# FlowEternal/multitask-hydranet

Measured on AMD Instinct MI355X. Metric: images/sec (fwd+bwd) HydraNet @ default res, 1/2/4/8 MI355X; CPU-ref same run, higher is better.
Workload: dtype bf16; 1 GPU; full HydraNet (backbone + BiFPN + seg/det/lane heads + multitask loss), big cfg, fwd+loss+bwd; batch_per_gpu=16, global_batch=16, resolution=3x512x1024, parallelism=dp1, hipgraph=True

## Files before the change

include/hydranet_hip.h:

```cpp
#ifndef HYDRANET_HIP_H
#define HYDRANET_HIP_H

#ifdef __cplusplus
extern "C" {
#endif

typedef struct ihipStream_t* hipStream_t;


int hn_gconv_pack_diag(const float* w, void* wk, void* wd, int C, hipStream_t stream);
int hn_pack_weight(const float* w, void* wp, void* wt, int Cout, int Cin, int taps, hipStream_t stream);
int hn_pack_weight_ex(const float* w, void* wp, void* wt, int Cout, int Cin_total, int ci0, int Cin, int taps, int phase, const float* bias,
                      float* b_eff, hipStream_t stream);
int hn_phase_fold(const float* dw_eff, const float* dw1, const float* db_eff, float* dw, float* db, int K, int C0, int C1, hipStream_t stream);
int hn_pack_weights_batched(const long* jobs, int njobs, long total_blocks, const int* block_job, hipStream_t stream);
int hn_pack_small_batched(const long* jobs, const int* block_job, long total_blocks, hipStream_t stream);

int hn_conv_gemm_nt(const void* x0, const void* x1, int mode, int n_img, int H, int W, int C0, int C1, int ld0, int ld1, int up, long M,
                    const void* w, int Nout, int KP, int taps, const float* bias, int act, void* out, int out_f32, int ldc, long rpi,
                    long img_stride, float* psum, float* psq, hipStream_t stream);
int hn_nt_stat_rows(long M, int Nout);
int hn_nt_stat_tile(long M, int Nout);
int hn_direct_stat_rows(int n_img, int H, int W);
int hn_conv_gemm_nt_imgw(const void* x0, int ld0, long M, int C0, const void* w, long w_img_stride, long rows_per_image, int Nout, int KP,
                         const float* bias, int act, void* out, int ldc, const void* addend, int ld_add, hipStream_t stream);
int hn_scale_weight_gate(const void* wp, const float* gate, void* out, int N, int Cout, int C, int KP, hipStream_t stream);
int hn_conv_gemm_nt_lvl(const void* x0, int ld0, long M, int C0, const void* w, int Nout, int KP, const float* bias, int act, void* out,
                        int ldc, const float* coef, int nlev, const long* rows, hipStream_t stream);
int hn_conv_gemm_nt_lvlout(const void* x0, int ld0, long M, int C0, const void* w, int Nout, int KP, const float* bias, int act, float* out,
                           int ldc, long img_stride, int n_img, int nlev, const int* H, const int* W, int row_align, hipStream_t stream);

int hn_conv_gemm_nt_ex(const void* x0, const void* x1, int mode, int n_img, int H, int W, int C0, int C1, int ld0, int ld1, int up, long M,
                       const void* w, int Nout, int KP, int taps, const float* bias, int act, void* out, int out_f32, int ldc, long rpi,
                       long img_stride, float* psum, float* psq, const float* xscale, const float* xshift, const float* xgate, long xhw,
                       int xact, const void* addend, int ld_add, int add_mode, hipStream_t stream);
int hn_conv_gemm_nt_stat(const void* x0, const void* x1, int mode, int n_img, int H, int W, int C0, int C1, int ld0, int ld1, int up, long M,
                         const void* w, int Nout, int KP, int taps, const float* bias, int act, void* out, int out_f32, int ldc, long rpi,
                         long img_stride, float* psum, float* psq, const void* addend, int ld_add, int add_mode, int emode, const void* ez,
                         int ld_ez, const float* ecoef, hipStream_t stream);
int hn_conv_gemm_nt_stat3(const void* x0, int ld0, long M, int C0, const void* w, int Nout, int KP, void* out, int ldc, float* psum, float* psq,
                          const void* addend, int ld_add, const void* ez, int ld_ez, const void* ey, int ld_ey, const float* ecoef,
                          hipStream_t stream);
int hn_wgrad_plan(int mode, int n_img, int H, int W, long M, int Nout, int KP, int taps, int* splits, long* rows_per_split, long* ws_bytes);
int hn_conv_gemm_tn(const void* x0, const void* x1, int mode, int n_img, int H, int W, int C0, int C1, int ld0, int ld1, int up, long M,
                    const void* dz, int ldz, int Nout, int KP, int taps, float* workspace, float* dw, hipStream_t stream);


int hn_stem_fwd(const float* x, const float* w, void* z, void* patches, int N, int H, int W, hipStream_t stream);

int hn_gconv_pack(const float* w, void* wk, void* wd, int C, int flip, hipStream_t stream);
int hn_gconv_fwd(const void* in, int ldi, const void* wk, void* out, int ldo, int N, int Hi, int Wi, int C, int stride, hipStream_t stream);
int hn_gconv_dgrad_s2(const void* dz, int ldz, const void* wd, void* dx, int ldx, int N, int Hi, int Wi, int C, hipStream_t stream);
long hn_wgrad_chunks(long pixels, long items);
int hn_gconv_wgrad(const void* x, int ldx, const void* dz, int ldz, float* part, int N, int Hi, int Wi, int C, int stride,
                   hipStream_t stream);

int hn_dw_pack(const float* w, void* wk, void* wkf, int C, hipStream_t stream);
int hn_dwconv_fwd(const void* in, int ldi, const void* wk, void* out, int ldo, int N, int H, int W, int C, hipStream_t stream);
int hn_dwconv_fwd_levels(const void* in, int ldi, const void* wk, void* out, int ldo, int N, int C, int nlev, const int* H, const int* W,
                         int row_align, int accumulate, hipStream_t stream);
long hn_dwconv_wgrad_blocks(long strips, int C);
int hn_dwconv_wgrad(const void* x, int ldx, const void* dz, int ldz, float* part, int N, int H, int W, int C, hipStream_t stream);
int hn_dwconv_wgrad_levels(const void* x, int ldx, const void* dz, int ldz, float* part, int N, int C, int nlev, const int* H, const int* W,
                           int row_align, hipStream_t stream);
long hn_dwconv_bwd_blocks(long strips, int C);
long hn_dwconv_bwd_blocks_levels(int N, int C, int nlev, const int* H, const int* W);
int hn_dwconv_bwd_levels(const void* dz, int ldz, const void* x, int ldx, const void* wf, void* dx, int lddx, float* part, int N, int C,
                         int nlev, const int* H, const int* W, int row_align, int accumulate, hipStream_t stream);

int hn_maxpool_fwd(const void* in, int ldi, void* out, int ldo, int N, int H, int W, int C, int mode, hipStream_t stream);
int hn_maxpool_bwd(const void* in, int ldi, const void* dout, int ldd, void* dx, int ldx, const float* wscale, int N, int H, int W, int C,
                   int mode, hipStream_t stream);
int hn_maxpool_bwd2(const void* in, int ldi, const void* dout, int ldd, void* dx, int ldx, const float* wscale, void* arg_ws, int N, int H,
                    int W, int C, int mode, int accumulate, hipStream_t stream);

int hn_up2_fwd(const void* in, int ldi, void* out, int ldo, int N, int H, int W, int C, hipStream_t stream);
int hn_sum2x2(const void* g, int ldg, void* out, int ldo, const float* wscale, int N, int H, int W, int C, int accumulate, hipStream_t stream);

int hn_fuse_dweights(const float* pw, int blocks, const float* praw, int nw, float eps, float* dp, hipStream_t stream);
int hn_fuse_fwd(const void* const* in, const int* ld, const int* mode, const float* w, void* out, int ldo, int N, int H, int W, int C,
                hipStream_t stream);
int hn_fuse_fwd_raw(const void* const* in, const int* ld, const int* mode, const float* praw, int nw, float eps, float* wn, void* out, int ldo,
                    int N, int H, int W, int C, hipStream_t stream);
int hn_fuse_bwd_blocks(int N, int H, int W, int C);
int hn_fuse_bwd(const void* const* in, const int* ld, const int* mode, const float* w, const void* dout, int ldd, void* g, int ldg,
                void* const* din, const int* ldin, const int* acc, float* pw, int N, int H, int W, int C, hipStream_t stream);
int hn_fuse_bwd_arg(const void* const* in, const int* ld, const int* mode, const float* w, const void* dout, int ldd, void* g, int ldg,
                    void* const* din, const int* ldin, const int* acc, float* pw, void* const* arg_out, int N, int H, int W, int C,
                    hipStream_t stream);
int hn_maxpool_bwd_from_arg(const void* arg, const void* dout, int ldd, void* dx, int ldx, const float* wscale, int N, int H, int W, int C,
                            int mode, int accumulate, hipStream_t stream);

long hn_fold_ring_rows(int H, int W);
int hn_conv3x3_dgrad_fold(const void* dz, int ldz, int Cz, int n_img, int H, int W, const void* wt, int Nout, int KP, int phase_k, int clamp,
                          void* out, int ldo, const void* yprev, int ldy, void* ring, hipStream_t stream);
int hn_conv3x3_dgrad_fold_s2d(const void* dz, int ldz, int Cz, int n_img, int H, int W, const void* wt, int Nout, int KP, int phase_k, int clamp,
                              void* out, int ldo, void* out_s2d, int ld_s2d, const void* yprev, int ldy, void* ring, hipStream_t stream);
int hn_seg_fold(const void* dvp, int ldv, int c0, void* out, int ldo, const void* yprev, int ldy, int N, int H, int W, int C, int up,
                hipStream_t stream);

int hn_space_to_depth(const float* dy, void* out, int ldo, int N, int h, int w, int k, hipStream_t stream);

int hn_space_to_depth_blocks(int N, int h, int w, int k);
int hn_space_to_depth_bf16(const void* in, int ldi, void* out, int N, int h, int w, int k, float* psum, hipStream_t stream);

int hn_conv3x3_phase(const void* x0, int mode, int n_img, int H, int W, int C0, int ld0, const void* w, int Nout, int KP, const float* bias,
                     int act, void* out, int ldc, int k, const void* addend, int ld_add, hipStream_t stream);
int hn_conv3x3_out_argmax(const void* x0, int n_img, int H, int W, int C0, int ld0, const void* w, int k, int KP, const float* bias, long* mask,
                          hipStream_t stream);
int hn_wgrad_plan_phase(int n_img, int H, int W, int Nout, int KP, int phase_span, int* splits, long* rows_per_split, long* ws_bytes);
int hn_conv_gemm_tn_phase(const void* x0, int n_img, int H, int W, int C0, int ld0, const void* dz, int ldz, int Nout, int KP, int phase_span,
                          float* workspace, float* dw, float* dbias_eff, hipStream_t stream);
int hn_conv_gemm_tn_deferred(const void* x0, const void* x1, int mode, int n_img, int H, int W, int C0, int C1, int ld0, int ld1, int up, long M,
                             const void* dz, int ldz, int Nout, int KP, int taps, float* workspace, float* dw, long* job, hipStream_t stream);
int hn_wgrad_reduce_jobs(const long* jobs, int njobs, hipStream_t stream);
long hn_gconv_wgrad_group_ws_bytes(const long* jobs, int njobs);
int hn_gconv_wgrad_group(const long* jobs, int njobs, float* workspace, hipStream_t stream);

int hn_grad_tail(const long* jobs, int njobs, hipStream_t stream);

long hn_wgrad_group_ws_bytes(const long* jobs, int njobs);
int hn_wgrad_group(const long* jobs, int njobs, float* workspace, hipStream_t stream);

int hn_conv_gemm_tn_bias(const void* x0, const void* x1, int mode, int n_img, int H, int W, int C0, int C1, int ld0, int ld1, int up, long M,
                         const void* dz, int ldz, int Nout, int KP, int taps, float* workspace, float* dw, float* dbias, hipStream_t stream);

int hn_head_grad(const float* dy, const float* y, long rpi, long img_stride, int lds, int Nout, void* dz, int ldz, long M, int sigmoid,
                 hipStream_t stream);

int hn_pack_levels(const void* const* src, const int* ld, void* dst, int ldd, int N, int C, int nlev, const int* H, const int* W, int row_align,
                   hipStream_t stream);
int hn_head_grad_levels(const float* dy, const float* y, long img_stride, int lds, int Nout, void* dz, int ldz, int N, int nlev, const int* H,
                        const int* W, int row_align, int sigmoid, hipStream_t stream);


long hn_colred_rows(long M, long align);
int hn_col_stats(const void* x, int ldx, long M, int C, long R, float* psum, float* psq, hipStream_t stream);
int hn_col_dot(const void* a, int lda, const void* b, int ldb, long M, int C, long R, float* pdot, float* psum, hipStream_t stream);
int hn_rows_reduce(const float* in, float* out, int G, int S, int C, float alpha, hipStream_t stream);
int hn_rows_reduce2(const float* in1, const float* in2, float* out1, float* out2, int rows, int G, int C, hipStream_t stream);

int hn_bn_finalize(const float* psum, const float* psq, int prows, int C, long count, const float* gamma, const float* beta, float eps,
                   float momentum, float* running_mean, float* running_var, float* scale, float* shift, float* mean, float* rstd,
                   hipStream_t stream);
int hn_bn_eval_coeff(const float* gamma, const float* beta, const float* rm, const float* rv, float eps, int C, float* scale, float* shift,
                     hipStream_t stream);
int hn_bn_act(const void* z, int ldz, const float* scale, const float* shift, const void* res, int ldr, const float* rscale,
              const float* rshift, int act, void* out, int ldo, long M, int C, hipStream_t stream);
int hn_bn_bwd_reduce(const void* dout, int ldd, const void* z, int ldz, const void* y, int ldy, const float* scale, const float* shift,
                     const float* mean, const float* rstd, int act, long M, int C, long R, float* pg, float* pgx, hipStream_t stream);
int hn_bn_bwd_finalize(const float* pg, const float* pgx, int prows, int C, long count, float* dgamma, float* dbeta, float* mg, float* mgx,
                       hipStream_t stream);
int hn_bn_bwd_apply(const void* dout, int ldd, const void* z, int ldz, const void* y, int ldy, const float* scale, const float* shift,
                    const float* mean, const float* rstd, const float* mg, const float* mgx, int act, void* dz, int lddz, void* gout, int ldg,
                    long M, int C, hipStream_t stream);

dgamma/dbeta are HOST arrays of nlev device pointers.  Partial-row inputs hold one row per `div` tensor rows. */
int hn_bn_finalize_levels(const float* psum, const float* psq, int div, int C, int nlev, const long* rows, const long* count,
                          const void* const* gamma, const void* const* beta, void* const* running_mean, void* const* running_var, float eps,
                          float momentum, const float* conv_bias, float* coef, hipStream_t stream);
int hn_bn_act_levels(const void* z, int ldz, const float* coef, int act, void* out, int ldo, int C, int nlev, const long* rows,
                     hipStream_t stream);
int hn_bn_bwd_reduce_levels(const void* dout, int ldd, const void* z, int ldz, const void* y, int ldy, const float* coef, int act, int C,
                            long R, int nlev, const long* rows, float* pg, float* pgx, hipStream_t stream);
int hn_bn_bwd_finalize_levels(const float* pg, const float* pgx, int div, int C, int nlev, const long* rows, const long* count,
                              void* const* dgamma, void* const* dbeta, float* red, float* zero_c, hipStream_t stream);
int hn_bn_bwd_apply_levels(const void* dout, int ldd, const void* z, int ldz, const void* y, int ldy, const float* coef, const float* red,
                           int act, void* dz, int lddz, int C, int nlev, const long* rows, hipStream_t stream);

long hn_fused_row_block(long M, int C, long align, int P, int kind);
int hn_bn_apply_fused(const void* z, int ldz, long M, int C, const float* psum, const float* psq, int P, long count, const float* gamma,
                      const float* beta, float eps, float momentum, float* rm, float* rv, float* coef, const void* res, int ldr, int act,
                      void* out, int ldo, float* pool, const float* gate, long HW, long RB, hipStream_t stream);
int hn_se_gate_apply(const void* z, int ldz, const float* coef, int act, const float* hid, const float* w2, const float* b2, float* gate,
                     void* out, int ldo, int N, long HW, int C, int Cs, hipStream_t stream);
// ... 272 lines not shown
```

multitask_hydranet_amd/_lib.py:

```python
from __future__ import annotations

import ctypes
import os
import re
import subprocess
from typing import Dict, List, Tuple

_PKG = os.path.dirname(os.path.abspath(__file__))
_ROOT = os.path.dirname(_PKG)
HEADER = os.path.join(_ROOT, "include", "hydranet_hip.h")
CSRC = os.path.join(_PKG, "csrc")
TUNING = os.environ.get("HN_TUNING") == "1"
AB = TUNING or os.environ.get("HN_TUNING") == "ab"


def policy(name: str, default: str) -> str:
    return os.environ.get(name, default) if AB else default

SO_PATH = os.path.join(_PKG, "libhydranet_hip_tuning.so" if TUNING else "libhydranet_hip.so")
SOURCES = ["hn_gemm.hip", "hn_norm.hip", "hn_fused.hip", "hn_stencil.hip", "hn_loss.hip", "hn_lovasz.hip", "hn_post.hip", "hn_xstage.hip", "hn_coco.hip",
           "hn_lane_encode.hip", "hn_augment.hip", "hn_jpeg.hip", "hn_jpeg_enc.hip", "hn_jpeg_huff.hip", "hn_jpeg_scan.hip", "hn_draw.hip", "hn_lane_metric.hip", "hn_png.hip", "hn_png_enc.hip",
           "hn_lane_filter.hip", "hn_state.hip", "hn_accum.hip", "hn_ckpt.hip", "hn_det_loss.hip", "hn_det_atss.hip", "hn_det_tal.hip", "hn_lane_liou.hip"]

_ERR = {1: "bad argument", 2: "kernel launch failure", 3: "unsupported shape"}


class HipKernelError(RuntimeError):
    pass


def _ctype(decl: str):
    decl = decl.strip()
    if "*" in decl or "hipStream_t" in decl:
        return ctypes.c_void_p
    words = decl.replace("const", " ").split()
    base = words[0]
    return {"int": ctypes.c_int, "long": ctypes.c_long, "float": ctypes.c_float, "double": ctypes.c_double}[base]


TUNING_HEADER = os.path.join(_ROOT, "include", "hydranet_hip_tuning.h")


def parse_header(path: str = HEADER) -> Dict[str, Tuple[object, List[object], bool]]:
    txt = open(path).read()
    if TUNING and path == HEADER:
        txt += open(TUNING_HEADER).read()
    txt = re.sub(r"/\*.*?\*/", " ", txt, flags=re.S)
    out = {}
    for m in re.finditer(r"\b(int|long)\s+(hn_\w+)\s*\((.*?)\)\s*;", txt, flags=re.S):
        ret, name, params = m.group(1), m.group(2), m.group(3)
        plist = [p for p in (q.strip() for q in params.replace("\n", " ").split(",")) if p and p != "void"]
        args = [_ctype(p) for p in plist]
        out[name] = (ctypes.c_int if ret == "int" else ctypes.c_long, args, bool(plist) and "hipStream_t" in plist[-1])
    return out


def sources() -> List[str]:
    return [os.path.join(CSRC, s) for s in SOURCES if os.path.exists(os.path.join(CSRC, s))]


def build(force: bool = False, verbose: bool = False) -> str:
    srcs = sources()
    deps = srcs + [os.path.join(CSRC, "hn_common.h"), os.path.join(CSRC, "hn_jpeg_tables.h"), os.path.join(CSRC, "hn_jpeg_scan.h"),
                   os.path.join(CSRC, "hn_det_common.h")]
    if not force and os.path.exists(SO_PATH) and all(os.path.getmtime(SO_PATH) >= os.path.getmtime(d) for d in deps):
        return SO_PATH
    hipcc = os.environ.get("HIPCC", "/opt/rocm/bin/hipcc")
    objs = []
    procs = []
    for s in srcs:
        o = os.path.join(CSRC, os.path.basename(s).replace(".hip", ".tuning.o" if TUNING else ".o"))
        objs.append(o)
        cmd = [hipcc, "--offload-arch=gfx950", "-O3", "-fPIC", "-std=c++17"] + (["-DHN_TUNING"] if TUNING else []) + ["-c", s, "-o", o]
        if verbose:
            print(" ".join(cmd))
        procs.append((cmd, subprocess.Popen(cmd, stdout=subprocess.PIPE, stderr=subprocess.STDOUT)))
    for cmd, p in procs:
        outp = p.communicate()[0].decode()
        if p.returncode != 0:
            raise RuntimeError("hipcc failed: %s\n%s" % (" ".join(cmd), outp))
    cmd = [hipcc, "--offload-arch=gfx950", "-shared", "-fPIC", "-o", SO_PATH] + objs
    r = subprocess.run(cmd, stdout=subprocess.PIPE, stderr=subprocess.STDOUT)
    if r.returncode != 0:
        raise RuntimeError("link failed: %s\n%s" % (" ".join(cmd), r.stdout.decode()))
    return SO_PATH


class _Lib:
    def __init__(self):
        if not os.path.exists(SO_PATH):
            raise HipKernelError(
                f"{SO_PATH} is missing: build it with `python -c 'import __graft_entry__ as g; g.build()'` "
                "(there is no CPU / eager fallback for the HydraNet hot path)")
        self._dll = ctypes.CDLL(policy("HN_LIB_AB", "") or SO_PATH)
        self._sig = parse_header()
        self._fn = {}
        for name, (ret, args, has_stream) in self._sig.items():
            f = getattr(self._dll, name)
            f.restype = ret
            f.argtypes = args
            self._fn[name] = (f, has_stream)

    def symbols(self):
        return sorted(self._sig)

    def raw(self, name):
        return self._fn[name][0]

    def call(self, name, *args):
        import torch
        f, has_stream = self._fn[name]
        if has_stream:
            args = args + (torch.cuda.current_stream().cuda_stream,)
        rc = f(*args)
        if rc != 0:
            raise HipKernelError(f"{name} failed: {_ERR.get(rc, rc)} (args={args})")

    def query(self, name, *args):
        if name not in self._fn and name.startswith("hn_debug_"):
            raise HipKernelError(f"{name} exists only in the tuning build of the library: set HN_TUNING=1 before importing the package "
                                 "(tools/ only; the product library has no tuning hooks)")
        return self._fn[name][0](*args)


_LIB = None


def lib() -> _Lib:
    global _LIB
    if _LIB is None:
        _LIB = _Lib()
    return _LIB
```

multitask_hydranet_amd/ops/core.py:

```python
from __future__ import annotations

import ctypes
import os
from typing import Optional, Sequence, Tuple

import torch

from .._lib import lib, policy

ACT_NONE, ACT_RELU, ACT_SWISH, ACT_ELU, ACT_SIGMOID = 0, 1, 2, 3, 4
GCONV_MFMA = True
BF16 = torch.bfloat16
F32 = torch.float32



def ptr(t: Optional[torch.Tensor]):
    return None if t is None else t.data_ptr()


def ld(t: torch.Tensor) -> int:
    assert t.dim() == 4 and (t.stride(3) == 1 or t.shape[3] == 1), (t.shape, t.stride())
    n, h, w, c = t.shape
    if w > 1:
# ... 120 lines not shown
            nb = (elements + 255) // 256
            row[6] = sblk[0]
            small_rows.append(row + [0] * (16 - len(row)))
            small_owner.extend([len(small_rows) - 1] * nb)
            sblk[0] += nb

        for key, w, meta in entries:
            kind = key[0] if isinstance(key, tuple) else key
            if kind == "conv":
                cout, cin = w.shape[0], w.shape[1]
                taps = w.shape[2] * w.shape[3]
                assert taps in (1, 9)
                wp = torch.empty((cout, taps * kp32(cin)), device=dev, dtype=BF16)
                wt = torch.empty((cin, taps * kp32(cout)), device=dev, dtype=BF16)
                dense_rows.append([w.data_ptr(), wp.data_ptr(), wt.data_ptr(), cout, cin, taps, dblk, kp32(cin) // 32])
                nb = (kp32(cout) // 32) * (kp32(cin) // 32)
                dense_owner += [len(dense_rows) - 1] * nb
                dblk += nb
                self.values.append((wp, wt))
            elif kind == "dw":
                c = w.shape[0]
                wk, wf = torch.empty((9 * c,), device=dev, dtype=BF16), torch.empty((9 * c,), device=dev, dtype=BF16)
                small([w.data_ptr(), wk.data_ptr(), wf.data_ptr(), 0, 0, 1, 0, c], 9 * c)
                self.values.append((wk, wf))
            elif kind == "g":
                c, flip = w.shape[0], key[1]
                wk, wd = torch.empty((72 * c,), device=dev, dtype=BF16), torch.empty((72 * c,), device=dev, dtype=BF16)
                small([w.data_ptr(), wk.data_ptr(), wd.data_ptr(), 0, 0, 2, 0, c // 8, flip], 72 * c)
                self.values.append((wk, wd))
            elif kind == "gdiag":
                c = w.shape[0]
                wk, wd = torch.zeros((c, 576), device=dev, dtype=BF16), torch.zeros((c, 576), device=dev, dtype=BF16)
                small([w.data_ptr(), wk.data_ptr(), wd.data_ptr(), 0, 0, 3, 0, c], 72 * c)
                self.values.append((wk, wd))
            elif kind in ("slice", "phase"):
                cout, cin_total, taps = w.shape[0], w.shape[1], w.shape[2] * w.shape[3]
                phase = 1 if kind == "phase" else 0
                ci0, cin = (0, key[1]) if phase else (key[1], key[2])
                coute = 4 * cout if phase else cout
                wp = torch.empty((coute, taps * kp32(cin)), device=dev, dtype=BF16)
                wt = torch.empty((cin, taps * kp32(coute)), device=dev, dtype=BF16) if (not phase or key[2]) else None
                b_eff = torch.empty((coute,), device=dev, dtype=F32) if phase else None
                bias = meta if phase else None
                small([w.data_ptr(), wp.data_ptr(), wt.data_ptr() if wt is not None else 0, b_eff.data_ptr() if phase else 0,
                       bias.data_ptr() if phase else 0, 4, 0, cout, cin_total, ci0, cin, taps, phase],
                      wp.numel() // 8 + (wt.numel() // 8 if wt is not None else 0) + (coute if phase else 0))
                self.values.append((wp, wt, b_eff, bias) if phase else (wp, wt))
            else:
                raise KeyError(key)
        self.dense_blocks, self.small_blocks = dblk, sblk[0]
        mk = lambda rows_, dt: torch.tensor(rows_, dtype=dt).to(dev) if rows_ else None
        self.dense_table, self.dense_owner = mk(dense_rows, torch.int64), mk(dense_owner, torch.int32)
        self.small_table, self.small_owner = mk(small_rows, torch.int64), mk(small_owner, torch.int32)
        self.n_dense = len(dense_rows)
        self.device = dev
        self._ran = None
        self.ptrs = [(w.data_ptr(), meta.data_ptr() if isinstance(meta, torch.Tensor) else 0) for _, w, meta in entries]

    @property
    def packs(self):
        return [v for (key, _, _), v in zip(self.entries, self.values) if key == "conv"]

    def valid(self):
        return all(w.data_ptr() == p_[0] and w.device == self.device and (not isinstance(meta, torch.Tensor) or meta.data_ptr() == p_[1])
                   for (_, w, meta), p_ in zip(self.entries, self.ptrs))

    def _versions(self):
        return (mutation_epoch(self.entries[0][1] if self.entries else None),
                [(w._version, meta._version if isinstance(meta, torch.Tensor) else 0) for _, w, meta in self.entries])

    def fresh(self):
        return self._ran == self._versions() and all(_PACK_CACHE.get((key, id(w)), (None,))[0] is w for key, w, _ in self.entries)

    def run(self):
        self._ran = self._versions()
        if self.dense_table is not None:
            lib().call("hn_pack_weights_batched", ptr(self.dense_table), self.n_dense, self.dense_blocks, ptr(self.dense_owner))
        if self.small_table is not None:
            lib().call("hn_pack_small_batched", ptr(self.small_table), ptr(self.small_owner), self.small_blocks)
        for (key, w, meta), v in zip(self.entries, self.values):
            if isinstance(key, tuple) and key[0] == "phase":
                v = (v[0], v[1], v[2], meta, meta._version)
            _PACK_CACHE[(key, id(w))] = (w, w._version, v)


def pack_conv_weight(w: torch.Tensor):
    def make():
        cout, cin = w.shape[0], w.shape[1]
        taps = w.shape[2] * w.shape[3]
        wp = torch.empty((cout, taps * kp32(cin)), device=w.device, dtype=BF16)
        wt = torch.empty((cin, taps * kp32(cout)), device=w.device, dtype=BF16)
        lib().call("hn_pack_weight", ptr(w), ptr(wp), ptr(wt), cout, cin, taps)
        return wp, wt
    return _cached("conv", w, make)


def pack_conv_weight_slice(w: torch.Tensor, ci0: int, cin: int):
    def make():
        cout, taps = w.shape[0], w.shape[2] * w.shape[3]
        wp = torch.empty((cout, taps * kp32(cin)), device=w.device, dtype=BF16)
        wt = torch.empty((cin, taps * kp32(cout)), device=w.device, dtype=BF16)
        lib().call("hn_pack_weight_ex", ptr(w), ptr(wp), ptr(wt), cout, w.shape[1], ci0, cin, taps, 0, None, None)
        return wp, wt
    return _cached(("slice", ci0, cin), w, make)


def pack_phase_weight(w: torch.Tensor, c0: int, bias: torch.Tensor, want_wt: bool = True):
    key = ("phase", c0, 1 if want_wt else 0)

    def make():
        k = w.shape[0]
        wp = torch.empty((4 * k, 9 * kp32(c0)), device=w.device, dtype=BF16)
        wt = torch.empty((c0, 9 * kp32(4 * k)), device=w.device, dtype=BF16) if want_wt else None
        b_eff = torch.empty((4 * k,), device=w.device, dtype=F32)
        lib().call("hn_pack_weight_ex", ptr(w), ptr(wp), ptr(wt), k, w.shape[1], 0, c0, 9, 1, ptr(bias), ptr(b_eff))
        return wp, wt, b_eff, bias, bias._version
    v = _cached(key, w, make, meta=bias)
    if v[3] is not bias or v[4] != bias._version:
        _PACK_CACHE.pop((key, id(w)), None)
        v = _cached(key, w, make, meta=bias)
    return v[0], v[1], v[2]


def pack_gconv_weight(w: torch.Tensor, flip: int):
    def make():
        c = w.shape[0]
        wk = torch.empty((9 * 8 * c,), device=w.device, dtype=BF16)
        wd = torch.empty((9 * 8 * c,), device=w.device, dtype=BF16)
        lib().call("hn_gconv_pack", ptr(w), ptr(wk), ptr(wd), c, flip)
        return wk, wd
    return _cached(("g", flip), w, make)


def pack_gconv_diag(w: torch.Tensor):
    def make():
        c = w.shape[0]
        wk = torch.empty((c, 9 * 64), device=w.device, dtype=BF16)
        wd = torch.empty((c, 9 * 64), device=w.device, dtype=BF16)
        lib().call("hn_gconv_pack_diag", ptr(w), ptr(wk), ptr(wd), c)
        return wk, wd
    return _cached("gdiag", w, make)


def pack_dw_weight(w: torch.Tensor):
    def make():
        c = w.shape[0]
        wk = torch.empty((9 * c,), device=w.device, dtype=BF16)
        wf = torch.empty((9 * c,), device=w.device, dtype=BF16)
        lib().call("hn_dw_pack", ptr(w), ptr(wk), ptr(wf), c)
        return wk, wf
    return _cached("dw", w, make)


def k_gemm_nt(x0, x1, mode, grid, wp, nout, kp, taps, bias=None, act=ACT_NONE, out=None, out_f32=False, up=0, stats=False,
              c0=None, c1=None, rpi=0, img_stride=0, ldc=None, xform=None, addend=None, add_pre=False, add_s2=False, estat=None):
    n, h, w = grid
    m = n * h * w
    dev = x0.device
    c0 = x0.shape[3] if c0 is None else c0
    c1 = (x1.shape[3] if x1 is not None else 0) if c1 is None else c1
    if out is None:
        out = torch.empty((n, h, w, nout), device=dev, dtype=F32 if out_f32 else BF16)
    if ldc is None:
        ldc = out.stride(2) if out.dim() == 4 else nout
    psum = psq = None
    if stats or estat is not None:
        pr = lib().query("hn_direct_stat_rows", n, h, w) if mode == 5 else lib().query("hn_nt_stat_rows", m, nout)
        psum = torch.empty((pr, nout), device=dev, dtype=F32)
        psq = torch.empty((pr, nout), device=dev, dtype=F32) if (estat is None or estat[0] != 1) else None
    if estat is not None:
        assert xform is None and not add_pre
        emode, ez, ecoef = estat[:3]
        if emode == 3:
            ey = estat[3]
            assert mode == 0 and taps == 1 and addend is not None and not add_s2 and x1 is None and not out_f32
            lib().call("hn_conv_gemm_nt_stat3", ptr(x0), ld(x0), m, c0, ptr(wp), nout, kp, ptr(out), ldc, ptr(psum), ptr(psq), ptr(addend),
                       ld(addend), ptr(ez), ld(ez), ptr(ey), ld(ey), ptr(ecoef))
            return out, psum, psq
        lib().call("hn_conv_gemm_nt_stat", ptr(x0), ptr(x1), mode, n, h, w, c0, c1, ld(x0), ld(x1) if x1 is not None else 0, up, m,
                   ptr(wp), nout, kp, taps, ptr(bias), act, ptr(out), 0, ldc, rpi, img_stride, ptr(psum), ptr(psq), ptr(addend),
                   ld(addend) if addend is not None else 0, 1 if add_s2 else 0, emode, ptr(ez), ld(ez), ptr(ecoef))
    elif xform is None and addend is None:
        lib().call("hn_conv_gemm_nt", ptr(x0), ptr(x1), mode, n, h, w, c0, c1, ld(x0), ld(x1) if x1 is not None else 0, up, m,
                   ptr(wp), nout, kp, taps, ptr(bias), act, ptr(out), 1 if out_f32 else 0, ldc, rpi, img_stride, ptr(psum), ptr(psq))
    else:
        xs, xh, xg, xhw, xact = xform if xform is not None else (None, None, None, 0, 0)
        lib().call("hn_conv_gemm_nt_ex", ptr(x0), ptr(x1), mode, n, h, w, c0, c1, ld(x0), ld(x1) if x1 is not None else 0, up, m,
                   ptr(wp), nout, kp, taps, ptr(bias), act, ptr(out), 1 if out_f32 else 0, ldc, rpi, img_stride, ptr(psum), ptr(psq),
                   ptr(xs), ptr(xh), ptr(xg), xhw, xact, ptr(addend),
                   (-ld(addend) if add_pre else ld(addend)) if addend is not None else 0, 1 if add_s2 else 0)
    return out, psum, psq


def wgrad_bias_ok(mode, kp):
    return mode != 5


class WgradBatch:

    def __init__(self):
        self.jobs = (ctypes.c_long * 32)()
        self.n = 0
        self.keep = []

    def slot(self, ws):
        assert self.n < 4
        self.keep.append(ws)
        self.n += 1
        return ctypes.addressof(self.jobs) + 64 * (self.n - 1)

    def flush(self):
        if self.n:
            lib().call("hn_wgrad_reduce_jobs", ctypes.addressof(self.jobs), self.n)
        self.n = 0
        self.keep = []


DEFER_WGRAD = policy("HN_DEFER_WGRAD", "1") != "0"


class GradQueue:
    MAX_GEMM = 32
    MAX_TAIL = 64

    def __init__(self):
        self.weights = ()
        self.jobs = []
        self.gconv = []
        self.tail = []

    def add(self, weight, x0, dz, mode, grid, cin, nout):
        self.jobs.append((weight, x0, dz, mode, grid, cin, nout))

    add_gemm = add

    def add_gconv(self, weight, x, dz, grid, c):
        self.gconv.append((weight, x, dz, grid, c))

    def add_rows(self, weight, part, rows, cols, shape):
        self.tail.append(((weight,), 0, part, None, rows, cols, 0, (shape,)))

    def add_fuse(self, praw, pw, blocks, eps):
        self.tail.append(((praw,), 1, pw, praw, blocks, praw.numel(), ctypes.c_uint.from_buffer(ctypes.c_float(eps)).value, (tuple(praw.shape),)))

    def add_outer(self, weight, bias, p, q):
        self.tail.append(((weight, bias), 2, p, q, p.shape[1], q.shape[1], p.shape[0], (tuple(weight.shape), tuple(bias.shape))))

    def flush(self):
        jobs, self.jobs = self.jobs, []
        tail, self.tail = self.tail, []
        gconv, self.gconv = self.gconv, []
        out = {}
        taken = set()

        def put(wgt, g):
            out[id(wgt)] = g if id(wgt) not in out else out[id(wgt)] + g
        for c0 in range(0, len(jobs), self.MAX_GEMM):
            chunk = jobs[c0:c0 + self.MAX_GEMM]
            tab = (ctypes.c_long * (12 * len(chunk)))()
            dws = []
            for i, (wgt, x0, dz, mode, (n, h, w), cin, nout) in enumerate(chunk):
                dw = grad_out(wgt, (nout, cin, 1, 1), dz.device, taken)
                dws.append(dw)
                ldz = dz.stride(2) if dz.dim() == 4 else dz.stride(0)
                tab[12 * i:12 * i + 12] = [x0.data_ptr(), dz.data_ptr(), dw.data_ptr(), mode, n, h, w, cin, ld(x0), ldz, nout, n * h * w]
            wsb = lib().query("hn_wgrad_group_ws_bytes", ctypes.addressof(tab), len(chunk))
            if wsb < 0:
                raise RuntimeError("hn_wgrad_group: bad job table")
            ws = torch.empty((wsb // 4,), device=chunk[0][2].device, dtype=F32)
            lib().call("hn_wgrad_group", ctypes.addressof(tab), len(chunk), ptr(ws))
            for (wgt, *_), dw in zip(chunk, dws):
                put(wgt, dw)
        for c0 in range(0, len(gconv), self.MAX_GEMM):
            chunk = gconv[c0:c0 + self.MAX_GEMM]
            tab = (ctypes.c_long * (9 * len(chunk)))()
            dws = []
            for i, (wgt, x, dz, (n, h, w), c) in enumerate(chunk):
                dw = grad_out(wgt, (c, 8, 3, 3), dz.device, taken)
                dws.append(dw)
                tab[9 * i:9 * i + 9] = [x.data_ptr(), dz.data_ptr(), dw.data_ptr(), n, h, w, c, ld(x), ld(dz)]
            wsb = lib().query("hn_gconv_wgrad_group_ws_bytes", ctypes.addressof(tab), len(chunk))
            if wsb < 0:
                raise RuntimeError("hn_gconv_wgrad_group: bad job table")
            ws = torch.empty((wsb // 4,), device=chunk[0][2].device, dtype=F32)
            lib().call("hn_gconv_wgrad_group", ctypes.addressof(tab), len(chunk), ptr(ws))
            for (wgt, *_), dw in zip(chunk, dws):
                put(wgt, dw)
        for c0 in range(0, len(tail), self.MAX_TAIL):
            chunk = tail[c0:c0 + self.MAX_TAIL]
            tab = (ctypes.c_long * (8 * len(chunk)))()
            done = []
            for i, (wts, kind, a, b, n0, n1, n2, shapes) in enumerate(chunk):
                outs = [grad_out(wgt, shp, a.device, taken) for wgt, shp in zip(wts, shapes)]
                tab[8 * i:8 * i + 8] = [kind, a.data_ptr(), b.data_ptr() if b is not None else 0, outs[0].data_ptr(),
                                        outs[1].data_ptr() if len(outs) > 1 else 0, n0, n1, n2]
                done += list(zip(wts, outs))
            lib().call("hn_grad_tail", ctypes.addressof(tab), len(chunk))
            for wgt, g in done:
                put(wgt, g)
        return [out.get(id(w)) for w in self.weights]


def grad_out(wgt, shape, dev, taken):
    slot = getattr(wgt, "_hn_grad_slot", None)
    if slot is not None and wgt.grad is None and id(wgt) not in taken:
        flat, off = slot
        n = 1
        for d in shape:
            n *= d
        if flat.device == dev and flat.dtype == F32:
            taken.add(id(wgt))
            return flat[off:off + n].view(shape)
    return torch.empty(shape, device=dev, dtype=F32)


WgradGroup = GradQueue
_CUR_QUEUE = None


def set_queue(q):
    global _CUR_QUEUE
    _CUR_QUEUE = q


def cur_queue():
    return _CUR_QUEUE if DEFER_WGRAD else None


SIDE_FLUSH = policy("HN_SIDE_FLUSH", "0") == "1"
_SIDE = {}


def _side_state(dev):
    st = _SIDE.get(dev)
# ... 238 lines not shown
```

Baseline: 981.3 images/sec.

## Add persistent streaming GEMM kernel for small-K 1x1 convs with LDS-resident weights

Adds a persistent kernel for eligible 1x1 conv GEMMs, with the grid capped at twice the CU count. Each block loads the weight tile into LDS once and streams 64-row activation tiles through a 2–3 slot multi-buffer using global_load_lds. Bias, activation and optional BN partial stats are fused into the epilogue, and output is staged through LDS for coalesced stores. The Python dispatcher sends matching calls to it by default: mode 0, one tap, no extra inputs, K≤128, 64<Nout≤128, and rows in a mid-size range. This targets launch/tail overhead and exposed load latency of the generic NT GEMM on bandwidth-bound layers. The risk is that the per-64-row psum layout may not match the row count the caller allocated for statistics.

```diff
diff --git a/include/hydranet_hip.h b/include/hydranet_hip.h
--- a/include/hydranet_hip.h
+++ b/include/hydranet_hip.h
@@ -21,6 +21,9 @@
                     long img_stride, float* psum, float* psq, hipStream_t stream);
 int hn_nt_stat_rows(long M, int Nout);
 int hn_nt_stat_tile(long M, int Nout);
+int hn_conv_gemm_nt_stream(const void* x, int ld0, long M, int C0, const void* w, int Nout, int KP, const float* bias, int act, void* out,
+                           int ldc, float* psum, float* psq, int wg_limit, hipStream_t stream);
+int hn_nt_stream_ok(long M, int C0, int Nout, int KP);
 int hn_direct_stat_rows(int n_img, int H, int W);
 int hn_conv_gemm_nt_imgw(const void* x0, int ld0, long M, int C0, const void* w, long w_img_stride, long rows_per_image, int Nout, int KP,
                          const float* bias, int act, void* out, int ldc, const void* addend, int ld_add, hipStream_t stream);
diff --git a/multitask_hydranet_amd/_lib.py b/multitask_hydranet_amd/_lib.py
--- a/multitask_hydranet_amd/_lib.py
+++ b/multitask_hydranet_amd/_lib.py
@@ -20,7 +20,8 @@
 SO_PATH = os.path.join(_PKG, "libhydranet_hip_tuning.so" if TUNING else "libhydranet_hip.so")
 SOURCES = ["hn_gemm.hip", "hn_norm.hip", "hn_fused.hip", "hn_stencil.hip", "hn_loss.hip", "hn_lovasz.hip", "hn_post.hip", "hn_xstage.hip", "hn_coco.hip",
            "hn_lane_encode.hip", "hn_augment.hip", "hn_jpeg.hip", "hn_jpeg_enc.hip", "hn_jpeg_huff.hip", "hn_jpeg_scan.hip", "hn_draw.hip", "hn_lane_metric.hip", "hn_png.hip", "hn_png_enc.hip",
-           "hn_lane_filter.hip", "hn_state.hip", "hn_accum.hip", "hn_ckpt.hip", "hn_det_loss.hip", "hn_det_atss.hip", "hn_det_tal.hip", "hn_lane_liou.hip"]
+           "hn_lane_filter.hip", "hn_state.hip", "hn_accum.hip", "hn_ckpt.hip", "hn_det_loss.hip", "hn_det_atss.hip", "hn_det_tal.hip", "hn_lane_liou.hip",
+           "hn_gemm_stream.hip"]
 
 _ERR = {1: "bad argument", 2: "kernel launch failure", 3: "unsupported shape"}
 
diff --git a/multitask_hydranet_amd/csrc/hn_gemm_stream.hip b/multitask_hydranet_amd/csrc/hn_gemm_stream.hip
--- /dev/null
+++ b/multitask_hydranet_amd/csrc/hn_gemm_stream.hip
@@ -0,0 +1,232 @@
+#include "hn_common.h"
+
+static __device__ __attribute__((aligned(16))) bf16 g_stream_zero_piece[8];
+
+__device__ __forceinline__ void glds16s(const bf16* src, char* lds_wave_base) {
+    __builtin_amdgcn_global_load_lds((const __attribute__((address_space(1))) void*)src,
+                                     (__attribute__((address_space(3))) void*)lds_wave_base, 16, 0, 0);
+}
+__device__ __forceinline__ int swz256(int row, int piece) { return row * 256 + ((piece ^ (row & 15)) << 4); }
+
+struct GemmStream {
+    const bf16* x; int ld0, C0; long M;
+    const bf16* w; int Nout, KP;
+    const float* bias; int act;
+    bf16* out; int ldc;
+    float* psum; float* psq;
+    int tiles;
+};
+
+#define HN_STREAM_XT (64 * 256)
+#define HN_STREAM_NT 512
+#define HN_STREAM_LPT 2
+
+#define HN_STREAM_BARRIER() asm volatile("s_waitcnt lgkmcnt(0)\n\ts_barrier" ::: "memory")
+
+template <int NB>
+__global__ __launch_bounds__(HN_STREAM_NT, 2) void gemm_nt_stream_kernel(const GemmStream p) {
+    constexpr int TC = 2, TP = 2, WC = 32, WP = 32, BC = 128;
+    extern __shared__ __attribute__((aligned(16))) char smem[];
+    const int tid = threadIdx.x, lane = tid & 63, wave = __builtin_amdgcn_readfirstlane(tid >> 6);
+    const int wc = wave >> 1, wp = wave & 1;
+    const int wrows = (p.Nout + 15) & ~15;
+    char* sWt = smem;
+    char* sX0 = smem + wrows * 256;
+    float* red = reinterpret_cast<float*>(sX0 + NB * HN_STREAM_XT);
+
+    const int G = gridDim.x, NG = G < 8 ? G : 8;
+    const int grp = blockIdx.x % NG, j0 = blockIdx.x / NG, ngrp = (G - grp + NG - 1) / NG;
+    const int t_lo = (int)((long)p.tiles * grp / NG), t_hi = (int)((long)p.tiles * (grp + 1) / NG);
+    int t_cur = t_lo + j0;
+    if (t_cur >= t_hi) return;
+
+    const int r0 = tid >> 4, lp = (tid & 15) ^ (r0 & 15), ch = lp * 8;
+    const bool xcv = ch < p.C0, wcv = ch < p.KP;
+    auto issue_x = [&](int tile, int slot) {
+        char* sX = sX0 + slot * HN_STREAM_XT;
+#pragma unroll
+        for (int i = 0; i < HN_STREAM_LPT; ++i) {
+            const long m = (long)tile * 64 + r0 + 32 * i;
+            const bf16* src = (xcv && m < p.M) ? p.x + m * p.ld0 + ch : g_stream_zero_piece;
+            glds16s(src, sX + (wave * 4 + 32 * i) * 256);
+        }
+    };
+    float pbias[TC][4];
+#pragma unroll
+    for (int i = 0; i < TC; ++i) {
+        const int co0 = wc * WC + i * 16 + (lane >> 4) * 4;
+#pragma unroll
+        for (int r = 0; r < 4; ++r) pbias[i][r] = (p.bias && co0 + r < p.Nout) ? p.bias[co0 + r] : 0.f;
+    }
+    for (int i = 0; i < (wrows + 31) / 32; ++i) {
+        const int co = r0 + 32 * i;
+        const bf16* src = (wcv && co < p.Nout) ? p.w + (long)co * p.KP + ch : g_stream_zero_piece;
+        if (wave * 4 + 32 * i < wrows) glds16s(src, sWt + (wave * 4 + 32 * i) * 256);
+    }
+    int t_iss = t_cur, n_iss = 0;
+#pragma unroll
+    for (int s = 0; s < NB - 1; ++s) {
+        if (t_iss < t_hi) { issue_x(t_iss, s); t_iss += ngrp; ++n_iss; }
+    }
+#pragma unroll
+    for (int i = 0; i < TC; ++i)
+#pragma unroll
+        for (int r = 0; r < 4; ++r) asm volatile("" : "+v"(pbias[i][r]));
+    const int ksteps = p.KP >> 5;
+    const bool want_stats = p.psum != nullptr;
+    int slot = 0, slot_iss = NB - 1;
+
+    for (; t_cur < t_hi; t_cur += ngrp) {
+        HN_STREAM_BARRIER();
+        if (t_iss < t_hi) { issue_x(t_iss, slot_iss); t_iss += ngrp; ++n_iss; }
+        slot_iss = slot_iss + 1 == NB ? 0 : slot_iss + 1;
+        if (NB >= 3 && n_iss >= 3) asm volatile("s_waitcnt vmcnt(%0)\n\ts_barrier" ::"n"(2 * HN_STREAM_LPT) : "memory");
+        else if (n_iss >= 2) asm volatile("s_waitcnt vmcnt(%0)\n\ts_barrier" ::"n"(HN_STREAM_LPT) : "memory");
+        else asm volatile("s_waitcnt vmcnt(0)\n\ts_barrier" ::: "memory");
+        --n_iss;
+
+        char* sX = sX0 + slot * HN_STREAM_XT;
+        f32x4 acc[TC][TP];
+#pragma unroll
+        for (int i = 0; i < TC; ++i)
+#pragma unroll
+            for (int j = 0; j < TP; ++j) acc[i][j] = (f32x4){0.f, 0.f, 0.f, 0.f};
+        for (int ks = 0; ks < ksteps; ++ks) {
+            bf16x8 a[TC], b[TP];
+            const int piece = ks * 4 + (lane >> 4);
+#pragma unroll
+            for (int i = 0; i < TC; ++i)
+                if (wc * WC + i * 16 < p.Nout) a[i] = *reinterpret_cast<const bf16x8*>(sWt + swz256(wc * WC + i * 16 + (lane & 15), piece));
+#pragma unroll
+            for (int j = 0; j < TP; ++j) b[j] = *reinterpret_cast<const bf16x8*>(sX + swz256(wp * WP + j * 16 + (lane & 15), piece));
+#pragma unroll
+            for (int i = 0; i < TC; ++i)
+                if (wc * WC + i * 16 < p.Nout) {
+#pragma unroll
+                    for (int j = 0; j < TP; ++j) acc[i][j] = __builtin_amdgcn_mfma_f32_16x16x32_bf16(a[i], b[j], acc[i][j], 0, 0, 0);
+                }
+        }
+        if (ksteps & 1) {
+            const bf16x8 z = zero8();
+#pragma unroll
+            for (int i = 0; i < TC; ++i)
+#pragma unroll
+                for (int j = 0; j < TP; ++j) acc[i][j] = __builtin_amdgcn_mfma_f32_16x16x32_bf16(z, z, acc[i][j], 0, 0, 0);
+        }
+
+        const long p_blk = (long)t_cur * 64;
+        float vv[TC * TP * 4];
+#pragma unroll
+        for (int i = 0; i < TC; ++i)
+#pragma unroll
+            for (int j = 0; j < TP; ++j)
+#pragma unroll
+                for (int r = 0; r < 4; ++r) vv[(i * TP + j) * 4 + r] = acc[i][j][r] + pbias[i][r];
+        HN_STREAM_BARRIER();
+        if (want_stats) {
+#pragma unroll
+            for (int i = 0; i < TC; ++i) {
+                float s1[4] = {0.f, 0.f, 0.f, 0.f}, s2[4] = {0.f, 0.f, 0.f, 0.f};
+#pragma unroll
+                for (int j = 0; j < TP; ++j) {
+                    const bool pv = p_blk + wp * WP + j * 16 + (lane & 15) < p.M;
+#pragma unroll
+                    for (int r = 0; r < 4; ++r) {
+                        float q = bfround(vv[(i * TP + j) * 4 + r]);
+                        q = pv ? q : 0.f;
+                        s1[r] += q;
+                        s2[r] += q * q;
+                    }
+                }
+#pragma unroll
+                for (int r = 0; r < 4; ++r) {
+                    s1[r] = row16_sum(s1[r]);
+                    s2[r] = row16_sum(s2[r]);
+                }
+                if ((lane & 15) == 0) {
+                    const int cl = wc * WC + i * 16 + (lane >> 4) * 4;
+#pragma unroll
+                    for (int r = 0; r < 4; ++r) { red[(wp * BC + cl + r) * 2] = s1[r]; red[(wp * BC + cl + r) * 2 + 1] = s2[r]; }
+                }
+            }
+        }
+        act_fwd_n(vv, p.act);
+#pragma unroll
+        for (int i = 0; i < TC; ++i) {
+            const int col = wc * WC + i * 16 + (lane >> 4) * 4;
+#pragma unroll
+            for (int j = 0; j < TP; ++j) {
+                const int prow_l = wp * WP + j * 16 + (lane & 15);
+                const float* v = vv + (i * TP + j) * 4;
+                bf16x4 t = {f2bf(v[0]), f2bf(v[1]), f2bf(v[2]), f2bf(v[3])};
+                *reinterpret_cast<bf16x4*>(sX + prow_l * 256 + ((((col >> 3) ^ prow_l) & 15) << 4) + ((col >> 2) & 1) * 8) = t;
+            }
+        }
+        HN_STREAM_BARRIER();
+        if (want_stats && tid < p.Nout) {
+            float t1 = 0.f, t2 = 0.f;
+#pragma unroll
+            for (int k = 0; k < 2; ++k) { t1 += red[(k * BC + tid) * 2]; t2 += red[(k * BC + tid) * 2 + 1]; }
+            p.psum[(long)t_cur * p.Nout + tid] = t1;
+            if (p.psq) p.psq[(long)t_cur * p.Nout + tid] = t2;
+        }
+#pragma unroll
+        for (int u = 0; u < 2; ++u) {
+            const int idx = tid + HN_STREAM_NT * u, row = idx >> 4, pc = idx & 15;
+            const long pix = p_blk + row;
+            const int co = pc * 8;
+            if (pix < p.M && co < p.Nout) {
+                const bf16x8 v = *reinterpret_cast<const bf16x8*>(sX + row * 256 + (((pc ^ row) & 15) << 4));
+                *reinterpret_cast<bf16x8*>(p.out + pix * p.ldc + co) = v;
+            }
+        }
+        slot = slot + 1 == NB ? 0 : slot + 1;
+    }
+}
+
+extern "C" int hn_nt_stream_ok(long M, int C0, int Nout, int KP) {
+    const long max_rows = g_hn_knob[4] > g_hn_knob[5] ? g_hn_knob[4] : g_hn_knob[5];
+    return M > 0 && M <= max_rows && KP > 0 && (KP & 31) == 0 && KP <= 128 && Nout > 64 && Nout <= 128 && (Nout & 7) == 0 && C0 > 0 &&
+           (C0 & 7) == 0 && C0 <= KP;
+}
+
+static size_t stream_lds(int Nout, int nb) { return (size_t)((Nout + 15) & ~15) * 256 + (size_t)nb * HN_STREAM_XT + 2 * 128 * 2 * sizeof(float); }
+
+static int stream_slots() {
+    static std::atomic<int> cache[64];
+    int dev = 0;
+    if (hipGetDevice(&dev) != hipSuccess || dev < 0 || dev >= 64) return 0;
+    int v = cache[dev].load(std::memory_order_acquire);
+    if (v == 0) {
+        int cus = 0;
+        if (hipDeviceGetAttribute(&cus, hipDeviceAttributeMultiprocessorCount, dev) != hipSuccess || cus <= 0) return 0;
+        v = 2 * cus;
+        cache[dev].store(v, std::memory_order_release);
+    }
+    return v;
+}
+
+extern "C" int hn_conv_gemm_nt_stream(const void* x, int ld0, long M, int C0, const void* w, int Nout, int KP, const float* bias, int act,
+                                      void* out, int ldc, float* psum, float* psq, int wg_limit, hipStream_t st) {
+    HN_CHECK_ARG(x && w && out && wg_limit >= 0 && (!psq || psum) && ld0 >= C0 && ldc >= Nout);
+    const auto a16 = [](const void* q) { return (reinterpret_cast<uintptr_t>(q) & 15) == 0; };
+    if (!hn_nt_stream_ok(M, C0, Nout, KP) || (ld0 & 7) || (ldc & 7) || !a16(x) || !a16(w) || !a16(out)) return HN_ERR_UNSUPPORTED;
+    GemmStream p;
+    p.x = (const bf16*)x; p.ld0 = ld0; p.C0 = C0; p.M = M;
+    p.w = (const bf16*)w; p.Nout = Nout; p.KP = KP;
+    p.bias = bias; p.act = act;
+    p.out = (bf16*)out; p.ldc = ldc;
+    p.psum = psum; p.psq = psq;
+    p.tiles = cdiv(M, 64);
+    const int slots = stream_slots();
+    if (slots <= 0) return HN_ERR_LAUNCH;
+    const int nb = 2 * stream_lds(Nout, 3) <= 160 * 1024 ? 3 : 2;
+    const size_t lds = stream_lds(Nout, nb);
+    static std::atomic<unsigned long long> optin{0};
+    if (!lds_optin(optin, {(const void*)gemm_nt_stream_kernel<2>, (const void*)gemm_nt_stream_kernel<3>})) return HN_ERR_LAUNCH;
+    int grid = wg_limit > 0 ? wg_limit : p.tiles;
+    if (grid > slots) grid = slots;
+    if (nb == 3) hipLaunchKernelGGL((gemm_nt_stream_kernel<3>), dim3(grid), dim3(HN_STREAM_NT), lds, st, p);
+    else hipLaunchKernelGGL((gemm_nt_stream_kernel<2>), dim3(grid), dim3(HN_STREAM_NT), lds, st, p);
+    HN_LAUNCH_CHECK();
+}
diff --git a/multitask_hydranet_amd/ops/core.py b/multitask_hydranet_amd/ops/core.py
--- a/multitask_hydranet_amd/ops/core.py
+++ b/multitask_hydranet_amd/ops/core.py
@@ -296,6 +296,24 @@
     return _cached("dw", w, make)
 
 
+NT_STREAM = policy("HN_NT_STREAM", "1") != "0"
+NT_STREAM_MAX_ROWS = 262144
+NT_STREAM_MIN_ROWS = 32768
+
+
+def nt_stream_ok(m: int, c0: int, nout: int, kp: int) -> bool:
+    return (0 < m <= NT_STREAM_MAX_ROWS and 0 < kp <= 128 and kp % 32 == 0 and 64 < nout <= 128 and nout % 8 == 0
+            and 0 < c0 <= kp and c0 % 8 == 0)
+
+
+def nt_stream_route(x0, x1, mode, taps, m, c0, nout, kp, out, out_f32, ldc, rpi, xform, addend) -> bool:
+    if not NT_STREAM or mode != 0 or taps != 1 or x1 is not None or out_f32 or rpi or xform is not None or addend is not None:
+        return False
+    if m < NT_STREAM_MIN_ROWS or not nt_stream_ok(m, c0, nout, kp):
+        return False
+    return ld(x0) % 8 == 0 and ldc % 8 == 0 and x0.data_ptr() % 16 == 0 and out.data_ptr() % 16 == 0
+
+
 def k_gemm_nt(x0, x1, mode, grid, wp, nout, kp, taps, bias=None, act=ACT_NONE, out=None, out_f32=False, up=0, stats=False,
               c0=None, c1=None, rpi=0, img_stride=0, ldc=None, xform=None, addend=None, add_pre=False, add_s2=False, estat=None):
     n, h, w = grid
@@ -324,6 +342,8 @@
         lib().call("hn_conv_gemm_nt_stat", ptr(x0), ptr(x1), mode, n, h, w, c0, c1, ld(x0), ld(x1) if x1 is not None else 0, up, m,
                    ptr(wp), nout, kp, taps, ptr(bias), act, ptr(out), 0, ldc, rpi, img_stride, ptr(psum), ptr(psq), ptr(addend),
                    ld(addend) if addend is not None else 0, 1 if add_s2 else 0, emode, ptr(ez), ld(ez), ptr(ecoef))
+    elif nt_stream_route(x0, x1, mode, taps, m, c0, nout, kp, out, out_f32, ldc, rpi, xform, addend):
+        lib().call("hn_conv_gemm_nt_stream", ptr(x0), ld(x0), m, c0, ptr(wp), nout, kp, ptr(bias), act, ptr(out), ldc, ptr(psum), ptr(psq), 0)
     elif xform is None and addend is None:
         lib().call("hn_conv_gemm_nt", ptr(x0), ptr(x1), mode, n, h, w, c0, c1, ld(x0), ld(x1) if x1 is not None else 0, up, m,
                    ptr(wp), nout, kp, taps, ptr(bias), act, ptr(out), 1 if out_f32 else 0, ldc, rpi, img_stride, ptr(psum), ptr(psq))
```

After: 991.7 images/sec, median of 6. +1.1%, better.
